# tnestmeyer/reflectance-filtering

Hardware: AMD Instinct MI355X
Metric: megapixels/sec joint-bilateral sigma_c=20 sigma_s=22 @1080p (higher is better)
Workload: dtype f32

## Files before the change

include/reflectance_filtering_debug.h:

```cpp
#ifndef REFLECTANCE_FILTERING_DEBUG_H
#define REFLECTANCE_FILTERING_DEBUG_H

#ifdef __cplusplus
extern "C" {
#endif

int rf_debug_option(const char *name, int value);

int rf_debug_clock_probe(unsigned long long *out2, int micros, void *stream);

const char *rf_debug_build_info(void);

int rf_debug_jbf_points_plan(int n_params, const double *sigma_space, int d, int joint_cn, int flags,
                             int total_points, int *out, int max_chunks);

int rf_debug_jbf_ragged_plan(int n, const int *heights, const int *widths, int joint_cn, int src_cn,
                             int d, double sigma_color, double sigma_space, int flags, int *out,
                             int cap);

int rf_debug_jbf_ragged_slab_plan(int n, const int *heights, const int *widths, int joint_cn,
                                  int src_cn, int d, double sigma_color, double sigma_space, int flags,
                                  int *out, int cap);

int rf_debug_jbf_two_wg_plan(int n, int h, int w, int joint_cn, int src_cn, int d, double sigma_color,
                             double sigma_space, int flags, int *out);

int rf_debug_jbf_two_wg_calls(void);

int rf_debug_jbf_tile_flags(void *stream, unsigned char *out, int cap);

int rf_debug_colorize_ragged_plan(int n, const int *heights, const int *widths, int *out, int cap);

int rf_debug_gf_ragged_plan(int n, const int *heights, const int *widths, int guide_cn, int src_cn,
                            int radius, int flags, int *out, int cap);

int rf_debug_gf_launch_chunk(int chunk, int h, int w, int src_cn, int float_kernels);

int rf_debug_png_plan(int n, const int *heights, const int *widths, int cn_in, int flags, int *out,
                      int cap);

#ifdef __cplusplus
}
#endif
#endif
```

reflectance_filtering_amd/_ffi.py:

```python
import ctypes
import os
import threading

_HERE = os.path.dirname(os.path.abspath(__file__))
LIB_PATH = os.path.join(_HERE, "librf_hip.so")

RF_OK, RF_E_BADARG, RF_E_UNSUPPORTED, RF_E_WORKSPACE, RF_E_HIP = 0, -1, -2, -3, -4
BORDER_CONSTANT, BORDER_REPLICATE, BORDER_REFLECT, BORDER_WRAP, BORDER_REFLECT_101 = range(5)
BORDER_DEFAULT = BORDER_REFLECT_101
JBF_TRUE_DIVISION = 1
JBF_FORCE_GENERIC = 2
JBF_GREY_AS_BGR = 4
GF_GREY_AS_BGR = 1
PNG_GREY_AS_RGB = 1
PNG_FLAG_GREY, PNG_FLAG_BAD_FILTER = 1, 2
CNN_NPARAMS = 4513
CNN_NPACKED = 4673
CNN_NCHW_RGB, CNN_NHWC_BGR = 0, 1
CNN_LAYOUTS = {"nchw_rgb": CNN_NCHW_RGB, "nhwc_bgr": CNN_NHWC_BGR}

EXPORTS = ("rf_version", "rf_last_error", "rf_shutdown", "rf_jbf_u8", "rf_gf_workspace_bytes",
           "rf_gf_u8", "rf_gf_ex_u8", "rf_cnn_reflectance_u8", "rf_cnn_pack_weights",
           "rf_cnn_reflectance_packed_u8", "rf_colorize_workspace_bytes",
           "rf_colorize_srgb_u8", "rf_whdr_f32", "rf_jbf_f32_workspace_bytes", "rf_jbf_f32",
           "rf_gf_f32_workspace_bytes", "rf_gf_f32", "rf_jbf_points_workspace_bytes",
           "rf_jbf_points_u8", "rf_jbf_points_ragged_workspace_bytes", "rf_jbf_points_ragged_u8",
           "rf_whdr_points_u8", "rf_jbf_ragged_workspace_bytes", "rf_jbf_ragged_u8",
           "rf_colorize_ragged_workspace_bytes", "rf_colorize_ragged_srgb_u8",
           "rf_gf_ragged_workspace_bytes", "rf_gf_ragged_u8", "rf_png_stream_bound",
           "rf_png_workspace_bytes", "rf_png_deflate_ragged_u8",
           "rf_png_unfilter_workspace_bytes", "rf_png_unfilter_ragged_u8",
           "rf_colorize_ragged_r8_srgb_u8", "rf_cnn_reflectance_f32",
           "rf_cnn_reflectance_packed_f32", "rf_jbf_release_scratch")

DEBUG_EXPORTS = ("rf_debug_option", "rf_debug_clock_probe", "rf_debug_build_info",
                 "rf_debug_jbf_points_plan", "rf_debug_jbf_ragged_plan",
                 "rf_debug_jbf_ragged_slab_plan", "rf_debug_jbf_two_wg_plan",
                 "rf_debug_jbf_two_wg_calls", "rf_debug_jbf_tile_flags",
                 "rf_debug_colorize_ragged_plan",
                 "rf_debug_gf_ragged_plan", "rf_debug_gf_launch_chunk", "rf_debug_png_plan")
RESULT_CHANGING_OPTIONS = ("jbf_stage_only", "gf_exp_skip")

_lib = None
_lock = threading.Lock()


class RFError(RuntimeError):
    """A librf_hip.so entry point returned a negative code."""


def load_library():
    global _lib
    with _lock:
# ... 93 lines not shown
        lib.rf_debug_clock_probe.restype = ci
        lib.rf_debug_build_info.argtypes = []
        lib.rf_debug_build_info.restype = ctypes.c_char_p
        lib.rf_debug_jbf_points_plan.argtypes = [ci, vp, ci, ci, ci, ci, vp, ci]
        lib.rf_debug_jbf_points_plan.restype = ci
        lib.rf_debug_jbf_ragged_plan.argtypes = [ci, vp, vp, ci, ci, ci, cd, cd, ci, vp, ci]
        lib.rf_debug_jbf_ragged_plan.restype = ci
        lib.rf_debug_jbf_ragged_slab_plan.argtypes = [ci, vp, vp, ci, ci, ci, cd, cd, ci, vp, ci]
        lib.rf_debug_jbf_ragged_slab_plan.restype = ci
        lib.rf_debug_jbf_two_wg_plan.argtypes = [ci, ci, ci, ci, ci, ci, cd, cd, ci, vp]
        lib.rf_debug_jbf_two_wg_plan.restype = ci
        lib.rf_debug_jbf_two_wg_calls.argtypes = []
        lib.rf_debug_jbf_two_wg_calls.restype = ci
        lib.rf_debug_jbf_tile_flags.argtypes = [vp, vp, ci]
        lib.rf_debug_jbf_tile_flags.restype = ci
        lib.rf_debug_colorize_ragged_plan.argtypes = [ci, vp, vp, vp, ci]
        lib.rf_debug_colorize_ragged_plan.restype = ci
        lib.rf_debug_gf_ragged_plan.argtypes = [ci, vp, vp, ci, ci, ci, ci, vp, ci]
        lib.rf_debug_gf_ragged_plan.restype = ci
        lib.rf_debug_gf_launch_chunk.argtypes = [ci, ci, ci, ci, ci]
        lib.rf_debug_gf_launch_chunk.restype = ci
        import sys
        for item in filter(None, os.environ.get("RF_DEBUG_OPTIONS", "").split(",")):
            name, _, value = item.partition("=")
            name = name.strip()
            try:
                number = int(value or 1)
            except ValueError:
                raise RFError("RF_DEBUG_OPTIONS: %r is not an integer (option %r)" % (value, name))
            if lib.rf_debug_option(name.encode(), number) < 0:
# ... 108 lines not shown
    return tuple(int(v) for v in out[1:]) if rc == 1 else None


def jbf_tile_flags(stream, tiles):
    import numpy as np
    lib = load_library()
    out = np.zeros(int(tiles), dtype=np.uint8)
    rc = lib.rf_debug_jbf_tile_flags(stream, out.ctypes.data, int(tiles))
    if rc < 0:
        check(rc, "rf_debug_jbf_tile_flags")
    if rc != int(tiles):
        raise RFError("rf_debug_jbf_tile_flags: %d bytes where %d tiles were asked for" % (rc, tiles))
    return out


def colorize_ragged_plan(sizes):
    import numpy as np
    lib = load_library()
    sizes = np.asarray(sizes, dtype=np.int64).reshape(-1, 2)
    n = sizes.shape[0]
    hs = np.ascontiguousarray(sizes[:, 0], dtype=np.int32)
    ws = np.ascontiguousarray(sizes[:, 1], dtype=np.int32)
    out = np.zeros(n + 2, dtype=np.int32)
    rc = lib.rf_debug_colorize_ragged_plan(n, hs.ctypes.data, ws.ctypes.data, out.ctypes.data, n + 2)
    if rc < 0:
        check(rc, "rf_debug_colorize_ragged_plan")
    return int(out[0]), int(out[1]), [int(v) for v in out[2:]]


def gf_ragged_plan(sizes, guide_cn, src_cn, radius, flags=0):
# ... 42 lines not shown
```

reflectance_filtering_amd/csrc/rf_api.hip:

```cpp
#include "rf_common.hpp"

#include <atomic>
#include <cstring>

#include "reflectance_filtering_debug.h"

namespace rf {

void jbf_shutdown();
void jbf_scratch_release();
void cnn_shutdown();
void gf_shutdown();

char *last_error_buf()
{
    static thread_local char buf[512] = "";
    return buf;
}

int fail(int code, const char *fmt, ...)
{
    va_list ap;
    va_start(ap, fmt);
    vsnprintf(last_error_buf(), 512, fmt, ap);
// ... 9 lines not shown

extern "C" int rf_debug_option(const char *name, int value)
{
    static const char *const names[] = {"gf_two_kernel",     "jbf_stage_only",
                                                      "jbf_compiler_loop", "jbf_tile64_only",
                                                      "jbf_tune",          "jbf_f32_untiled",
                                                      "cnn_lds_columns",   "gf_seg_rows",
                                                      "gf_one_stream",     "gf_force_two_streams",
                                                      "gf_guide_cache",    "gf_chained",        "gf_no_compact",
                                                      "gf_exp_skip",       "gf_stagger",        "gf_parts",
                                                      "gf_s1_cap",         "gf_s1_min_wgs",
                                                      "jbf_lookahead1",    "gf_s1_legacy_strips",
                                                      "gf_exact_all_flagged", "gf_cw_chan_run",   "gf_exact",
                                                      "jbf_no_msad",       "colorize_chunk_px",
                                                      "jbf_no_two_wg",     "jbf_vote_scan",
                                                      "jbf_no_dead_skip"};
    static_assert(sizeof(names) / sizeof(names[0]) == rf::kDbgCount, "one name per DebugOption");
    if (name)
        for (int i = 0; i < rf::kDbgCount; i++)
            if (std::strcmp(name, names[i]) == 0)
                return rf::g_debug[i].exchange(value < 0 ? 0 : value);
    return rf::fail(RF_E_BADARG, "rf_debug_option: unknown option '%s'", name ? name : "(null)");
}

__global__ void clock_probe_kernel(unsigned long long *out, unsigned long long ticks)
{
    if (threadIdx.x != 0)
        return;
    const unsigned long long r0 = __builtin_amdgcn_s_memrealtime();
    const unsigned long long c0 = __builtin_amdgcn_s_memtime();
    unsigned long long r1 = r0;
// ... 42 lines not shown
```

reflectance_filtering_amd/csrc/rf_common.hpp:

```cpp
#pragma once
#include <hip/hip_runtime.h>

#include <cstdarg>
#include <cstdint>
#include <cstdio>

#include "reflectance_filtering.h"

namespace rf {

char *last_error_buf();
int fail(int code, const char *fmt, ...);

#define RF_HIP_CHECK(expr)                                                                   \
    do {                                                                                     \
        hipError_t _e = (expr);                                                              \
        if (_e != hipSuccess)                                                                \
            return ::rf::fail(RF_E_HIP, "%s failed: %s (%s:%d)", #expr, hipGetErrorString(_e), \
                              __FILE__, __LINE__);                                           \
    } while (0)

__host__ __device__ inline int border_interpolate(int p, int len, int border)
{
    if ((unsigned)p < (unsigned)len)
// ... 69 lines not shown
    kDbgGfExpSkip,
    kDbgGfStagger,
    kDbgGfParts,
    kDbgGfS1Cap,
    kDbgGfS1MinWgs,
    kDbgJbfLookahead1,
    kDbgGfS1LegacyStrips,
    kDbgGfExactAllFlagged,
    kDbgGfCwChanRun,
    kDbgGfExact,
    kDbgJbfNoMsad,
    kDbgColorizeChunkPx,
    kDbgJbfNoTwoWg,
    kDbgJbfVoteScan,
    kDbgJbfNoDeadSkip,
    kDbgCount
};
int debug_get(int id);

}
```

reflectance_filtering_amd/csrc/rf_jbf.hip:

```cpp
#include <algorithm>
#include <atomic>
#include <mutex>
#include <vector>

#include "rf_jbf_common.hpp"
#include "rf_jbf_tables.hpp"
#include "rf_jbf_taploops.hpp"

namespace rf {
namespace {

constexpr int kTileW = 64;
constexpr int kMaxLds = 160 * 1024;
constexpr int kTlw2 = 144;
constexpr int kJbfMaxTiledR4 = 468;
constexpr int kJbfStageOnly = 0x1000, kJbfCompilerLoop = 0x2000, kJbfTile64Only = 0x4000;
constexpr int kJbfLookahead1 = 0x8000;
constexpr int kJbfNoMsad = 0x10000;
constexpr int kJbfVoteOnly = 0x20000;
constexpr int kJbfNoDeadSkip = 0x40000;

int jbf_debug_flags()
{
    return (debug_get(kDbgJbfStageOnly) ? kJbfStageOnly : 0) |
// ... 1074 lines not shown
    auto kern = jbf_slab_kernel<GREP, TLW, true>;
    RF_HIP_CHECK(hipFuncSetAttribute((const void *)kern, hipFuncAttributeMaxDynamicSharedMemorySize,
                                     kT64Lds));
    hipLaunchKernelGGL(kern, dim3((unsigned)ntiles), dim3(1024), kT64Lds, stream, joint, src, dst, 0,
                       0, jcn, scn, t.radius, border, t.d_lut, nz, t.d_hw, t.d_swsym, t.sw_len,
                       d_recs, 0, flags, s.crows_g, s.slab_g, s.crows_c, s.slab_c);
    return RF_OK;
}

int tile64x2_slab_rows(int nz, int grep, int tlw)
{
    const int rows = (kT64x2Lds - nz * grep * 4) / (tlw * 4);
    return rows >= 64 ? rows - 64 + 1 : 0;
}

template <int GREP, int TLW>
__global__ __launch_bounds__(1024, 8) void jbf_tile64x2_kernel(
    const uint8_t *__restrict__ joint, const uint8_t *__restrict__ src, uint8_t *__restrict__ dst,
    int h, int w, int jcn, int scn, int radius, int border, const float *__restrict__ lut, int nz,
    const int *__restrict__ hwtab, const float *__restrict__ swsym, int sw_len, int tiles_x,
    int tiles_per_img, int flags, int slab_rows, uint8_t *__restrict__ tile_flags)
{
    constexpr int NT = 1024, Q4 = TLW / 4, QW = 16;
    static_assert(TLW % 32 == 16, "row pitch keeps the rows of a half-wave on disjoint banks");
    extern __shared__ __align__(16) unsigned char smem[];
    int *flag_word = reinterpret_cast<int *>(smem);
    uint32_t *tile4 = reinterpret_cast<uint32_t *>(smem);
    const int tid = threadIdx.x;
    if (tid == 0)
        *flag_word = 3;
    __syncthreads();
    const int tile_id = xcd_contiguous_tile((int)blockIdx.x, (int)gridDim.x);
    const int img_idx = tile_id / tiles_per_img;
    const int t_in_img = tile_id - img_idx * tiles_per_img;
    const int tile_y0 = (t_in_img / tiles_x) * 64;
    const int tile_x0 = (t_in_img % tiles_x) * 64;
// ... 25 lines not shown
    if (tile_flags) {
        const int byte = __builtin_amdgcn_readfirstlane((int)tile_flags[tile_id]);
        if (byte & 1)
            return;
        grey_joint = (byte >> 1) & 1;
    }
    float *lut_g = reinterpret_cast<float *>(smem + kT64x2Lds - nz * GREP * 4);
    for (int i = tid; i < nz * GREP; i += NT)
        lut_g[i] = lut[i / GREP];
    const uint32_t lut_lane_addr = lds_addr(lut_g) + (uint32_t)(tid & (GREP - 1)) * 4u;
    const uint32_t tile_lane_addr = lds_addr(tile4) + (uint32_t)tx * 4u;
    const bool j1 = grey_joint != 0;
    const uint32_t j1_scale = (uint32_t)(jcn == 1 ? 1 : 3) * (GREP * 4u);
    uint32_t jc[kPix];
    float sum1[kPix][1], wsum[kPix];
    {
        uint32_t jv[4], sv[4];
        load_tile_quad(joint, src, img, border_interpolate(tile_y0 + ty, h, border), tile_x0 + 4 * tx, w, jcn,
                       scn, border, jv, sv);
#pragma unroll
        for (int p = 0; p < kPix; p++) {
            jc[p] = j1 ? (jv[p] & 0xffu) * j1_scale : jv[p] & 0x00ffffffu;
            sum1[p][0] = 0.f;
            wsum[p] = 0.f;
        }
    }
    const bool msad = !j1 && !(flags & kJbfNoMsad) && jbf_wave_takes_msad(jc);
    const bool live_wave =
        __builtin_amdgcn_readfirstlane(tile_y0 + (ty & ~3)) < h || (flags & kJbfNoDeadSkip) != 0;
    for (int i0 = -radius; i0 <= radius; i0 += slab_rows) {
        const int i1 = min(i0 + slab_rows - 1, radius);
        const int tlh = 64 + (i1 - i0);
        __syncthreads();
        for (int item = tid; item < tlh * Q4; item += NT) {
            const int ry = item / Q4, k = item - ry * Q4;
            const int gy = border_interpolate(tile_y0 + i0 + ry, h, border);
            uint32_t jv[4], sv[4];
            load_tile_quad(joint, src, img, gy, tile_x0 - r4 + 4 * k, w, jcn, scn, border, jv, sv);
#pragma unroll
            for (int u = 0; u < 4; u++) {
                const uint32_t jfield = j1 ? (jv[u] & 0xffu) * j1_scale : jv[u];
                tile4[ry * TLW + u * Q4 + k] = jfield | (sv[u] << 24);
            }
        }
        __syncthreads();
        if (!live_wave)
            continue;
        if (j1)
            jbf_tap_loop_grey4_la2<GREP, TLW, true, true>(lut_lane_addr, swsym, tile_lane_addr, jc, ty,
                                                          radius, r4, sw_len, hwtab, sum1, wsum, i0, i1, -i0);
        else if (msad)
            jbf_tap_loop_grey4_la2<GREP, TLW, false, true, true>(lut_lane_addr, swsym, tile_lane_addr, jc,
                                                                 ty, radius, r4, sw_len, hwtab, sum1, wsum,
                                                                 i0, i1, -i0);
        else
            jbf_tap_loop_grey4_la2<GREP, TLW, false, true>(lut_lane_addr, swsym, tile_lane_addr, jc, ty,
                                                           radius, r4, sw_len, hwtab, sum1, wsum, i0, i1,
// ... 4 lines not shown
    else
        store_quad<1, 3>(dst, img, tile_y0 + ty, tile_x0 + 4 * tx, h, w, sum1, wsum, flags);
}

struct TileFlagBuf {
    int dev;
    hipStream_t stream;
    uint8_t *p;
    size_t bytes;
};
std::mutex g_tf_mu;
std::vector<TileFlagBuf> g_tf;
std::vector<uint8_t *> g_tf_retired;
constexpr size_t kTileFlagStreams = 16;
std::atomic<int> g_two_wg_calls{0};

size_t tile_flag_bytes(size_t tiles)
{
    size_t b = 4096;
    while (b < tiles)
        b <<= 1;
    return b;
}

int get_tile_flags(int dev, hipStream_t stream, size_t tiles, uint8_t **out)
{
    *out = nullptr;
    std::lock_guard<std::mutex> lock(g_tf_mu);
    size_t at = g_tf.size();
    for (size_t i = 0; i < g_tf.size(); i++)
// ... 12 lines not shown
        return RF_OK;
    uint8_t *p = nullptr;
    {
        CaptureRelax relax;
        RF_HIP_CHECK(hipMalloc(&p, tile_flag_bytes(tiles)));
    }
    if (at < g_tf.size()) {
        g_tf_retired.push_back(g_tf[at].p);
        g_tf.erase(g_tf.begin() + at);
    }
    g_tf.push_back(TileFlagBuf{dev, stream, p, tile_flag_bytes(tiles)});
    *out = p;
    return RF_OK;
}

bool two_wg_choose(const JbfTables &t, int nz, int src_cn, int flags, int *slab_rows)
{
    *slab_rows = 0;
    if (debug_get(kDbgJbfNoTwoWg) || debug_get(kDbgJbfTune) ||
        (flags & (RF_JBF_FORCE_GENERIC | kJbfStageOnly | kJbfCompilerLoop | kJbfLookahead1)))
        return false;
    Tile64Shape shape;
    if (t.r4 > 36 || !tile64_choose(t, nz, src_cn, flags, &shape) || shape.tlw != 144 || shape.grep != 32)
        return false;
    *slab_rows = tile64x2_slab_rows(nz, 32, 144);
    return *slab_rows >= 8;
}

int launch_tile64x2(const JbfTables &t, int nz, int slab_rows, const uint8_t *joint, const uint8_t *src,
                    uint8_t *dst, int n, int h, int w, int jcn, int scn, int border, int flags,
                    hipStream_t stream, int rows, int cols, uint8_t *tile_flags)
{
    const int tiles_x = ceil_div(cols, 64), tiles_y = ceil_div(rows, 64);
    const long long blocks = (long long)tiles_x * tiles_y * n;
    auto kern = jbf_tile64x2_kernel<32, 144>;
    RF_HIP_CHECK(hipFuncSetAttribute((const void *)kern, hipFuncAttributeMaxDynamicSharedMemorySize,
                                     kT64x2Lds));
    hipLaunchKernelGGL(kern, dim3((unsigned)blocks), dim3(1024), kT64x2Lds, stream, joint, src, dst, h, w,
                       jcn, scn, t.radius, border, t.d_lut, nz, t.d_hw, t.d_swsym, t.sw_len, tiles_x,
                       tiles_x * tiles_y, flags, slab_rows, tile_flags);
    return RF_OK;
}

template <int CREP>
int launch_tile64_flagged(const JbfTables &t, int nz, int crows, const uint8_t *joint, const uint8_t *src,
                          uint8_t *dst, int n, int h, int w, int jcn, int border, int flags,
                          hipStream_t stream, int rows, int cols, const uint8_t *tile_flags)
{
    const int tiles_x = ceil_div(cols, 64), tiles_y = ceil_div(rows, 64);
    const long long blocks = (long long)tiles_x * tiles_y * n;
    auto kern = jbf_tile64_kernel<3, 32, CREP, 144, 64, false, true>;
    RF_HIP_CHECK(hipFuncSetAttribute((const void *)kern, hipFuncAttributeMaxDynamicSharedMemorySize,
                                     kT64Lds));
    hipLaunchKernelGGL(kern, dim3((unsigned)blocks), dim3(1024), kT64Lds, stream, joint, src, dst, h, w,
                       jcn, t.radius, border, t.d_lut, nz, t.d_hw, t.d_swsym, t.sw_len, tiles_x,
// ... 1 lines not shown
    return RF_OK;
}

int launch_two_wg(const JbfTables &t, int nz, const Tile64Shape &shape, int slab_rows,
                  const uint8_t *joint, const uint8_t *src, uint8_t *dst, int n, int h, int w, int jcn,
                  int scn, int border, int flags, hipStream_t stream, bool *done)
{
    *done = false;
    const Tile64Areas a = tile64_areas(t, nz, shape.grep, shape.crep, scn, flags, h, w);
    if (a.rows_main <= 0 || a.cols_main <= 0)
        return RF_OK;
    const long long blocks = (long long)ceil_div(a.cols_main, 64) * ceil_div(a.rows_main, 64) * n;
    if (!launch_fits(blocks, 1024))
        return fail(RF_E_UNSUPPORTED, "rf_jbf_u8: batch too large for one launch");
    uint8_t *tile_flags = nullptr;
    int rc = RF_OK;
    if (scn == 3 || jcn == 3) {
        if (int bad = get_tile_flags(t.device, stream, (size_t)blocks, &tile_flags))
            return bad;
        if (!tile_flags)
            return RF_OK;
        const int tiles_x = ceil_div(a.cols_main, 64), tiles_y = ceil_div(a.rows_main, 64);
        if (debug_get(kDbgJbfVoteScan) || !jbf_grey_map_serves(h, w, t.radius, border, tiles_x, tiles_y))
            rc = launch_tile64x2(t, nz, slab_rows, joint, src, dst, n, h, w, jcn, scn, border,
                                 flags | kJbfVoteOnly, stream, a.rows_main, a.cols_main, tile_flags);
        else
            rc = jbf_launch_grey_map(joint, src, n, h, w, jcn, scn, t.radius, border, stream, tiles_x, tiles_y,
                                     tile_flags);
    }
    if (rc == RF_OK && scn == 3)
        rc = shape.crep == 32 ? launch_tile64_flagged<32>(t, nz, shape.crows, joint, src, dst, n, h, w, jcn,
                                                          border, flags, stream, a.rows_main, a.cols_main,
                                                          tile_flags)
                              : launch_tile64_flagged<16>(t, nz, shape.crows, joint, src, dst, n, h, w, jcn,
                                                          border, flags, stream, a.rows_main, a.cols_main,
                                                          tile_flags);
    if (rc == RF_OK)
        rc = launch_tile64x2(t, nz, slab_rows, joint, src, dst, n, h, w, jcn, scn, border, flags, stream,
                             a.rows_main, a.cols_main, tile_flags);
    if (rc == RF_OK && (a.s32 || a.s16 || a.sx)) {
        if (scn == 3)
            rc = shape.crep == 32 ? launch_tile64_rows<3, 32, 32>(t, nz, shape.crows, joint, src, dst, n, h, w,
                                                                  jcn, border, flags, stream, true)
                                  : launch_tile64_rows<3, 32, 16>(t, nz, shape.crows, joint, src, dst, n, h, w,
                                                                  jcn, border, flags, stream, true);
        else
            rc = shape.crep == 32 ? launch_tile64_rows<1, 32, 32>(t, nz, shape.crows, joint, src, dst, n, h, w,
                                                                  jcn, border, flags, stream, true)
                                  : launch_tile64_rows<1, 32, 16>(t, nz, shape.crows, joint, src, dst, n, h, w,
                                                                  jcn, border, flags, stream, true);
    }
    *done = rc == RF_OK;
    if (*done)
        g_two_wg_calls.fetch_add(1, std::memory_order_relaxed);
    return rc;
}

}

void jbf_scratch_release()
{
    std::lock_guard<std::mutex> lock(g_tf_mu);
    for (const TileFlagBuf &b : g_tf)
        (void)hipFree(b.p);
    for (uint8_t *p : g_tf_retired)
        (void)hipFree(p);
    g_tf.clear();
    g_tf_retired.clear();
}

}

extern "C" int rf_debug_jbf_two_wg_calls(void)
{
    return rf::g_two_wg_calls.load(std::memory_order_relaxed) & 0x7fffffff;
}

extern "C" int rf_debug_jbf_tile_flags(void *stream_, unsigned char *out, int cap)
{
    using namespace rf;
    hipStream_t stream = (hipStream_t)stream_;
    if (cap < 0 || (!out && cap))
        return fail(RF_E_BADARG, "rf_debug_jbf_tile_flags: NULL out or a negative cap");
// ... 5 lines not shown
    const uint8_t *p = nullptr;
    size_t bytes = 0;
    {
        std::lock_guard<std::mutex> lock(g_tf_mu);
        for (const TileFlagBuf &b : g_tf)
            if (b.dev == dev && b.stream == stream)
                p = b.p, bytes = b.bytes;
    }
    if (bytes > (size_t)cap)
        bytes = (size_t)cap;
    if (bytes) {
        RF_HIP_CHECK(hipMemcpyAsync(out, p, bytes, hipMemcpyDeviceToHost, stream));
        RF_HIP_CHECK(hipStreamSynchronize(stream));
    }
    return (int)bytes;
}

extern "C" int rf_jbf_release_scratch(void)
{
    rf::jbf_scratch_release();
    return RF_OK;
}

extern "C" int rf_jbf_u8(const uint8_t *joint, const uint8_t *src, uint8_t *dst, int n, int h,
                         int w, int joint_cn, int src_cn, int d, double sigma_color,
                         double sigma_space, int border, int flags, void *stream_)
{
    using namespace rf;
    if (n == 0)
        return RF_OK;
// ... 265 lines not shown
    out[0] = out[1] = out[2] = out[3] = 0;
    int slab_rows = 0;
    Tile64Shape shape;
    if (t.r4 > kJbfMaxTiledR4 || !two_wg_choose(t, nz, src_cn, flags, &slab_rows) ||
        !tile64_choose(t, nz, src_cn, flags, &shape))
        return 0;
    const Tile64Areas a = tile64_areas(t, nz, shape.grep, shape.crep, src_cn, flags, h, w);
    const long long blocks = (long long)ceil_div(a.cols_main, 64) * ceil_div(a.rows_main, 64) * n;
    if (a.rows_main <= 0 || a.cols_main <= 0 || !launch_fits(blocks, 1024))
        return 0;
    out[0] = 1;
    out[1] = 64 + slab_rows - 1;
    out[2] = (int)blocks;
    out[3] = src_cn == 3 || joint_cn == 3 ? (int)tile_flag_bytes((size_t)blocks) : 0;
    return 1;
}

extern "C" int rf_jbf_ragged_u8(const uint8_t *joint, const uint8_t *src, uint8_t *dst, int n,
                                const int *heights, const int *widths, int joint_cn, int src_cn,
                                int d, double sigma_color, double sigma_space, int border, int flags,
                                void *workspace, size_t workspace_bytes, void *stream_)
{
    using namespace rf;
    const char *who = "rf_jbf_ragged_u8";
    if (n == 0)
        return RF_OK;
    if (!joint || !src || !dst)
        return fail(RF_E_BADARG, "%s: NULL image pointer", who);
    size_t px, tiles;
    if (int bad = ragged_check(who, n, heights, widths, joint_cn, src_cn, d, sigma_space, border,
// ... 91 lines not shown
```

reflectance_filtering_amd/csrc/rf_jbf_common.hpp:

```cpp
#pragma once
#include <cmath>
#include <vector>

#include "rf_common.hpp"

namespace rf {

constexpr int kJbfPublicFlags = RF_JBF_TRUE_DIVISION | RF_JBF_FORCE_GENERIC | RF_JBF_GREY_AS_BGR;
constexpr int kJbfMaxRadius = 4096;

inline double jbf_sigma(double sigma) { return sigma <= 0 ? 1 : sigma; }

inline int jbf_radius(int d, double sigma_space)
{
    const int radius = d <= 0 ? (int)std::lrint(sigma_space * 1.5) : d / 2;
    return radius < 1 ? 1 : radius;
}

inline int jbf_table_cn(int joint_cn, int flags)
{
    return joint_cn == 1 && (flags & RF_JBF_GREY_AS_BGR) ? 3 : joint_cn;
}
inline int jbf_kernel_cn(int joint_cn, int flags)
{
// ... 1 lines not shown
}

inline int jbf_check_format(const char *who, int joint_cn, int src_cn, int border)
{
    if ((joint_cn != 1 && joint_cn != 3) || (src_cn != 1 && src_cn != 3))
        return fail(RF_E_UNSUPPORTED, "%s: channels must be 1 or 3 (joint %d, src %d)", who,
                    joint_cn, src_cn);
    if (border < 0 || border > 4)
        return fail(RF_E_UNSUPPORTED, "%s: border type %d", who, border);
    return RF_OK;
}

bool jbf_grey_map_serves(int h, int w, int radius, int border, int tiles_x, int tiles_y);
int jbf_launch_grey_map(const uint8_t *joint, const uint8_t *src, int n, int h, int w, int jcn, int scn,
                        int radius, int border, hipStream_t stream, int tiles_x, int tiles_y,
                        uint8_t *tile_flags);

int jbf_colour_lut(int joint_cn, double sigma_color, std::vector<float> &lut);

void jbf_space_taps(int radius, double sigma_space, std::vector<int> &di, std::vector<int> &dj,
                    std::vector<float> &sw, std::vector<int> &hw);

__device__ inline uint32_t load_packed(const uint8_t *img, size_t pix, int cn)
{
    if (cn < 0)
        return (uint32_t)img[pix] * 0x010101u;
    const uint8_t *p = img + pix * cn;
    uint32_t v = p[0];
    if (cn == 3)
        v |= ((uint32_t)p[1] << 8) | ((uint32_t)p[2] << 16);
    return v;
// ... 16 lines not shown
```

reflectance_filtering_amd/csrc/rf_jbf_greymap.hip:

```cpp
#include "rf_jbf_common.hpp"

namespace rf {
namespace {

__host__ __device__ inline void border_span(int a, int b, int len, int border, int *lo, int *hi)
{
    int l = a > 0 ? a : 0, u = b < len - 1 ? b : len - 1;
    if (border == RF_BORDER_REFLECT || border == RF_BORDER_REFLECT_101) {
        const int delta = border == RF_BORDER_REFLECT_101;
        if (a < 0) {
            const int top = -a - 1 + delta;
            u = top > u ? (top < len - 1 ? top : len - 1) : u;
        }
        if (b >= len) {
            const int back = 2 * len - 1 - b - delta;
            l = back < l ? (back > 0 ? back : 0) : l;
        }
    }
    *lo = l;
    *hi = u;
}

constexpr int kMapCols = 10, kMapRows = 4, kMapColFirst = -2, kMapRowFirst = -1;
constexpr int kMapBatch = 4;
// ... 9 lines not shown

__device__ inline void load12(const uint8_t *p, uint32_t (&d)[3])
{
    __builtin_memcpy(&d[0], p, 4);
    __builtin_memcpy(&d[1], p + 4, 4);
    __builtin_memcpy(&d[2], p + 8, 4);
}

__device__ inline void load_row_end(const uint8_t *p, int npx, uint32_t (&d)[3])
{
    d[0] = d[1] = d[2] = 0u;
    for (int k = 0; k < 3 * npx; k++)
        d[k >> 2] |= (uint32_t)p[k] << (8 * (k & 3));
}

__global__ __launch_bounds__(256) void jbf_grey_map_clear_kernel(uint32_t *__restrict__ words, int nwords)
{
    const int i = (int)blockIdx.x * 256 + (int)threadIdx.x;
    if (i < nwords)
        words[i] = 0x02020202u;
}

template <bool SRC, bool JOINT>
__global__ __launch_bounds__(256) void jbf_grey_map_kernel(
    const uint8_t *__restrict__ joint, const uint8_t *__restrict__ src, int h, int w, int radius, int border,
    int tiles_x, int tiles_y, int blocks_x, int blocks_y, uint32_t *__restrict__ tile_words)
{
    __shared__ uint32_t acc[2 * kMapRows];
    const int tid = threadIdx.x, lane = tid & 63, wave = tid >> 6;
    if (tid < 2 * kMapRows)
        acc[tid] = 0u;
    const int gx = (int)(blockIdx.x % (unsigned)blocks_x);
    const int gy = (int)((blockIdx.x / (unsigned)blocks_x) % (unsigned)blocks_y);
    const int img_idx = (int)(blockIdx.x / ((unsigned)blocks_x * (unsigned)blocks_y));
    const int r4 = (radius + 3) & ~3;
    const int x = 256 * gx + 4 * lane;
    uint32_t cm[4] = {0u, 0u, 0u, 0u};
#pragma unroll
    for (int c = 0; c < kMapCols; c++) {
        const int tx = 4 * gx + kMapColFirst + c;
        if (tx < 0 || tx >= tiles_x)
            continue;
// ... 2 lines not shown
#pragma unroll
        for (int u = 0; u < 4; u++)
            cm[u] |= (x + u >= lo && x + u <= hi) ? 1u << c : 0u;
    }
    int ylo[kMapRows], yhi[kMapRows];
#pragma unroll
    for (int r = 0; r < kMapRows; r++) {
        const int ty = gy + kMapRowFirst + r;
        ylo[r] = 1, yhi[r] = 0;
        if (ty >= 0 && ty < tiles_y)
            border_span(64 * ty - radius, 64 * ty + 63 + radius, h, border, &ylo[r], &yhi[r]);
    }
    __syncthreads();
    uint32_t as[kMapRows] = {0u, 0u, 0u, 0u}, aj[kMapRows] = {0u, 0u, 0u, 0u};
    const size_t img = (size_t)img_idx * h * w;
    const bool active = (cm[0] | cm[1] | cm[2] | cm[3]) != 0u;
    if (active && w - x >= 4) {
        for (int i0 = 0; i0 < 16; i0 += kMapBatch) {
            const int y0 = 64 * gy + wave + 4 * i0;
            if (y0 >= h)
                break;
            uint32_t ds[kMapBatch][3], dj[kMapBatch][3];
#pragma unroll
            for (int k = 0; k < kMapBatch; k++) {
                const int yc = min(y0 + 4 * k, h - 1);
                const size_t at = (img + (size_t)yc * w + x) * 3;
                if (SRC)
                    load12(src + at, ds[k]);
                if (JOINT)
                    load12(joint + at, dj[k]);
            }
#pragma unroll
            for (int k = 0; k < kMapBatch; k++) {
                const int y = y0 + 4 * k;
                const uint32_t cs = SRC ? coloured_columns(ds[k], cm) : 0u;
                const uint32_t cj = JOINT ? coloured_columns(dj[k], cm) : 0u;
#pragma unroll
                for (int r = 0; r < kMapRows; r++)
                    if (y >= ylo[r] && y <= yhi[r])
                        as[r] |= cs, aj[r] |= cj;
            }
        }
    } else if (active) {
        for (int i = 0; i < 16; i++) {
            const int y = 64 * gy + wave + 4 * i;
            if (y >= h)
                break;
            const size_t at = (img + (size_t)y * w + x) * 3;
            uint32_t cs = 0u, cj = 0u, d[3];
            if (SRC) {
                load_row_end(src + at, w - x, d);
                cs = coloured_columns(d, cm);
            }
            if (JOINT) {
                load_row_end(joint + at, w - x, d);
                cj = coloured_columns(d, cm);
            }
#pragma unroll
            for (int r = 0; r < kMapRows; r++)
                if (y >= ylo[r] && y <= yhi[r])
                    as[r] |= cs, aj[r] |= cj;
        }
    }
#pragma unroll
    for (int r = 0; r < kMapRows; r++) {
        if (as[r])
            atomicOr(&acc[r], as[r]);
        if (aj[r])
            atomicOr(&acc[kMapRows + r], aj[r]);
    }
    __syncthreads();
// ... 25 lines not shown
            if (tx < 4 * gx + kMapColFirst || tx >= 4 * gx + kMapColFirst + kMapCols)
                return false;
    }
    for (int ty = 0; ty < tiles_y; ty++) {
        int lo, hi;
        border_span(64 * ty - radius, 64 * ty + 63 + radius, h, border, &lo, &hi);
        for (int gy = lo / 64; gy <= hi / 64; gy++)
            if (ty < gy + kMapRowFirst || ty >= gy + kMapRowFirst + kMapRows)
                return false;
    }
    return true;
}

int jbf_launch_grey_map(const uint8_t *joint, const uint8_t *src, int n, int h, int w, int jcn, int scn,
                        int radius, int border, hipStream_t stream, int tiles_x, int tiles_y,
                        uint8_t *tile_flags)
{
    const int blocks_x = ceil_div(w, 256), blocks_y = ceil_div(h, 64);
    const long long blocks = (long long)blocks_x * blocks_y * n;
    if (!launch_fits(blocks, 256))
        return fail(RF_E_UNSUPPORTED, "rf_jbf_u8: batch too large for one launch");
    const int nwords = (int)(((long long)tiles_x * tiles_y * n + 3) / 4);
    uint32_t *words = reinterpret_cast<uint32_t *>(tile_flags);
    hipLaunchKernelGGL(jbf_grey_map_clear_kernel, dim3((unsigned)ceil_div(nwords, 256)), dim3(256), 0, stream,
                       words, nwords);
    if (scn != 3 && jcn != 3)
        return RF_OK;
    auto kern = scn == 3 && jcn == 3 ? jbf_grey_map_kernel<true, true>
                : scn == 3           ? jbf_grey_map_kernel<true, false>
                                     : jbf_grey_map_kernel<false, true>;
    hipLaunchKernelGGL(kern, dim3((unsigned)blocks), dim3(256), 0, stream, joint, src, h, w, radius, border,
                       tiles_x, tiles_y, blocks_x, blocks_y, words);
    return RF_OK;
}

}
```

Before: 2727.

## Pack joint and source pixels into 32-bit texels during grey-map pass

The grey-map pre-pass, which already reads both 3-channel joint and source images, now also writes an intermediate buffer of 32-bit texels (joint BGR plus one source channel byte) with padded row pitch. The main two-workgroup tile kernel then fills its LDS tile from this buffer with aligned 16-byte loads instead of unaligned 3-byte-pixel gathers from two images. The aim is cheaper, vectorised tile staging. The cost is an extra global write pass in the pre-pass, a cached per-stream scratch allocation of up to 4 GB, and more code paths. It also changes the stage-only debug gating.

Result: no change. 2752 (median of 6 runs) (+0.9%).

```diff
diff --git a/include/reflectance_filtering_debug.h b/include/reflectance_filtering_debug.h
--- a/include/reflectance_filtering_debug.h
+++ b/include/reflectance_filtering_debug.h
@@ -29,6 +29,13 @@
 
 int rf_debug_jbf_tile_flags(void *stream, unsigned char *out, int cap);
 
+long long rf_debug_jbf_packed_plan(int n, int h, int w, int joint_cn, int src_cn, int d, double sigma_color,
+                                   double sigma_space, int border, int flags);
+
+int rf_debug_jbf_packed_calls(void);
+
+long long rf_debug_jbf_packed_texels(void *stream, unsigned int *out, long long cap);
+
 int rf_debug_colorize_ragged_plan(int n, const int *heights, const int *widths, int *out, int cap);
 
 int rf_debug_gf_ragged_plan(int n, const int *heights, const int *widths, int guide_cn, int src_cn,
diff --git a/reflectance_filtering_amd/_ffi.py b/reflectance_filtering_amd/_ffi.py
--- a/reflectance_filtering_amd/_ffi.py
+++ b/reflectance_filtering_amd/_ffi.py
@@ -37,6 +37,7 @@
                  "rf_debug_jbf_points_plan", "rf_debug_jbf_ragged_plan",
                  "rf_debug_jbf_ragged_slab_plan", "rf_debug_jbf_two_wg_plan",
                  "rf_debug_jbf_two_wg_calls", "rf_debug_jbf_tile_flags",
+                 "rf_debug_jbf_packed_plan", "rf_debug_jbf_packed_calls", "rf_debug_jbf_packed_texels",
                  "rf_debug_colorize_ragged_plan",
                  "rf_debug_gf_ragged_plan", "rf_debug_gf_launch_chunk", "rf_debug_png_plan")
 RESULT_CHANGING_OPTIONS = ("jbf_stage_only", "gf_exp_skip")
@@ -160,6 +161,12 @@
         lib.rf_debug_jbf_two_wg_calls.restype = ci
         lib.rf_debug_jbf_tile_flags.argtypes = [vp, vp, ci]
         lib.rf_debug_jbf_tile_flags.restype = ci
+        lib.rf_debug_jbf_packed_plan.argtypes = [ci, ci, ci, ci, ci, ci, cd, cd, ci, ci]
+        lib.rf_debug_jbf_packed_plan.restype = ctypes.c_longlong
+        lib.rf_debug_jbf_packed_calls.argtypes = []
+        lib.rf_debug_jbf_packed_calls.restype = ci
+        lib.rf_debug_jbf_packed_texels.argtypes = [vp, vp, ctypes.c_longlong]
+        lib.rf_debug_jbf_packed_texels.restype = ctypes.c_longlong
         lib.rf_debug_colorize_ragged_plan.argtypes = [ci, vp, vp, vp, ci]
         lib.rf_debug_colorize_ragged_plan.restype = ci
         lib.rf_debug_gf_ragged_plan.argtypes = [ci, vp, vp, ci, ci, ci, ci, vp, ci]
@@ -298,6 +305,29 @@
     return out
 
 
+def jbf_packed_plan(n, h, w, joint_cn, src_cn, d, sigma_color, sigma_space, border=None, flags=0):
+    lib = load_library()
+    rc = lib.rf_debug_jbf_packed_plan(int(n), int(h), int(w), int(joint_cn), int(src_cn), int(d),
+                                      float(sigma_color), float(sigma_space),
+                                      BORDER_DEFAULT if border is None else int(border), int(flags))
+    if rc < 0:
+        check(int(rc), "rf_debug_jbf_packed_plan")
+    return int(rc)
+
+
+def jbf_packed_texels(stream, n, h, w):
+    import numpy as np
+    lib = load_library()
+    wpad = (int(w) + 3) & ~3
+    out = np.zeros(int(n) * int(h) * wpad, dtype=np.uint32)
+    rc = lib.rf_debug_jbf_packed_texels(stream, out.ctypes.data, out.size)
+    if rc < 0:
+        check(int(rc), "rf_debug_jbf_packed_texels")
+    if rc != out.size:
+        return None
+    return np.ascontiguousarray(out.reshape(int(n), int(h), wpad)[:, :, :int(w)])
+
+
 def colorize_ragged_plan(sizes):
     import numpy as np
     lib = load_library()
diff --git a/reflectance_filtering_amd/csrc/rf_api.hip b/reflectance_filtering_amd/csrc/rf_api.hip
--- a/reflectance_filtering_amd/csrc/rf_api.hip
+++ b/reflectance_filtering_amd/csrc/rf_api.hip
@@ -47,7 +47,8 @@
                                                       "gf_exact_all_flagged", "gf_cw_chan_run",   "gf_exact",
                                                       "jbf_no_msad",       "colorize_chunk_px",
                                                       "jbf_no_two_wg",     "jbf_vote_scan",
-                                                      "jbf_no_dead_skip"};
+                                                      "jbf_no_dead_skip",  "jbf_no_packed",
+                                                      "jbf_packed_cap_kb"};
     static_assert(sizeof(names) / sizeof(names[0]) == rf::kDbgCount, "one name per DebugOption");
     if (name)
         for (int i = 0; i < rf::kDbgCount; i++)
diff --git a/reflectance_filtering_amd/csrc/rf_common.hpp b/reflectance_filtering_amd/csrc/rf_common.hpp
--- a/reflectance_filtering_amd/csrc/rf_common.hpp
+++ b/reflectance_filtering_amd/csrc/rf_common.hpp
@@ -107,6 +107,8 @@
     kDbgJbfNoTwoWg,
     kDbgJbfVoteScan,
     kDbgJbfNoDeadSkip,
+    kDbgJbfNoPacked,
+    kDbgJbfPackedCapKb,
     kDbgCount
 };
 int debug_get(int id);
diff --git a/reflectance_filtering_amd/csrc/rf_jbf.hip b/reflectance_filtering_amd/csrc/rf_jbf.hip
--- a/reflectance_filtering_amd/csrc/rf_jbf.hip
+++ b/reflectance_filtering_amd/csrc/rf_jbf.hip
@@ -1112,12 +1112,29 @@
     return rows >= 64 ? rows - 64 + 1 : 0;
 }
 
-template <int GREP, int TLW>
+__device__ inline void load_texel_quad(const uint32_t *row, int x_first, int w, int border, uint32_t (&t)[4])
+{
+    if (!row) {
+        t[0] = t[1] = t[2] = t[3] = 0u;
+    } else if (x_first >= 0 && x_first + 3 < w) {
+        const uint4 v = *reinterpret_cast<const uint4 *>(row + x_first);
+        t[0] = v.x, t[1] = v.y, t[2] = v.z, t[3] = v.w;
+    } else {
+#pragma unroll
+        for (int u = 0; u < 4; u++) {
+            const int gx = border_interpolate(x_first + u, w, border);
+            t[u] = gx < 0 ? 0u : row[gx];
+        }
+    }
+}
+
+template <int GREP, int TLW, bool PACKED = false>
 __global__ __launch_bounds__(1024, 8) void jbf_tile64x2_kernel(
     const uint8_t *__restrict__ joint, const uint8_t *__restrict__ src, uint8_t *__restrict__ dst,
     int h, int w, int jcn, int scn, int radius, int border, const float *__restrict__ lut, int nz,
     const int *__restrict__ hwtab, const float *__restrict__ swsym, int sw_len, int tiles_x,
-    int tiles_per_img, int flags, int slab_rows, uint8_t *__restrict__ tile_flags)
+    int tiles_per_img, int flags, int slab_rows, uint8_t *__restrict__ tile_flags,
+    const uint32_t *__restrict__ packed)
 {
     constexpr int NT = 1024, Q4 = TLW / 4, QW = 16;
     static_assert(TLW % 32 == 16, "row pitch keeps the rows of a half-wave on disjoint banks");
@@ -1173,6 +1190,8 @@
     const uint32_t j1_scale = (uint32_t)(jcn == 1 ? 1 : 3) * (GREP * 4u);
     uint32_t jc[kPix];
     float sum1[kPix][1], wsum[kPix];
+    const int wpad = (w + 3) & ~3;
+    const uint32_t *const pimg = PACKED ? packed + (size_t)img_idx * h * wpad : nullptr;
     {
         uint32_t jv[4], sv[4];
         load_tile_quad(joint, src, img, border_interpolate(tile_y0 + ty, h, border), tile_x0 + 4 * tx, w, jcn,
@@ -1184,22 +1203,40 @@
             wsum[p] = 0.f;
         }
     }
+    constexpr int kDry = NT / Q4, kDk = NT % Q4;
+    const int ry_first = tid / Q4, k_first = tid - ry_first * Q4;
     const bool msad = !j1 && !(flags & kJbfNoMsad) && jbf_wave_takes_msad(jc);
     const bool live_wave =
-        __builtin_amdgcn_readfirstlane(tile_y0 + (ty & ~3)) < h || (flags & kJbfNoDeadSkip) != 0;
+        (__builtin_amdgcn_readfirstlane(tile_y0 + (ty & ~3)) < h || (flags & kJbfNoDeadSkip) != 0) &&
+        !(flags & kJbfStageOnly);
     for (int i0 = -radius; i0 <= radius; i0 += slab_rows) {
         const int i1 = min(i0 + slab_rows - 1, radius);
         const int tlh = 64 + (i1 - i0);
         __syncthreads();
-        for (int item = tid; item < tlh * Q4; item += NT) {
-            const int ry = item / Q4, k = item - ry * Q4;
-            const int gy = border_interpolate(tile_y0 + i0 + ry, h, border);
-            uint32_t jv[4], sv[4];
-            load_tile_quad(joint, src, img, gy, tile_x0 - r4 + 4 * k, w, jcn, scn, border, jv, sv);
-#pragma unroll
-            for (int u = 0; u < 4; u++) {
-                const uint32_t jfield = j1 ? (jv[u] & 0xffu) * j1_scale : jv[u];
-                tile4[ry * TLW + u * Q4 + k] = jfield | (sv[u] << 24);
+        if (PACKED) {
+            static_assert(kTileW % 4 == 0 && Q4 * 4 == TLW, "quads of the tile start at multiples of four");
+            for (int ry = ry_first, k = k_first; ry < tlh;) {
+                const int gy = border_interpolate(tile_y0 + i0 + ry, h, border);
+                uint32_t t[4];
+                load_texel_quad(gy < 0 ? nullptr : pimg + (size_t)gy * wpad, tile_x0 - r4 + 4 * k, w, border, t);
+#pragma unroll
+                for (int u = 0; u < 4; u++)
+                    tile4[ry * TLW + u * Q4 + k] = j1 ? ((t[u] & 0xffu) * j1_scale) | (t[u] & 0xff000000u) : t[u];
+                k += kDk, ry += kDry;
+                if (k >= Q4)
+                    k -= Q4, ry++;
+            }
+        } else {
+            for (int item = tid; item < tlh * Q4; item += NT) {
+                const int ry = item / Q4, k = item - ry * Q4;
+                const int gy = border_interpolate(tile_y0 + i0 + ry, h, border);
+                uint32_t jv[4], sv[4];
+                load_tile_quad(joint, src, img, gy, tile_x0 - r4 + 4 * k, w, jcn, scn, border, jv, sv);
+#pragma unroll
+                for (int u = 0; u < 4; u++) {
+                    const uint32_t jfield = j1 ? (jv[u] & 0xffu) * j1_scale : jv[u];
+                    tile4[ry * TLW + u * Q4 + k] = jfield | (sv[u] << 24);
+                }
             }
         }
         __syncthreads();
@@ -1234,6 +1271,7 @@
 std::vector<uint8_t *> g_tf_retired;
 constexpr size_t kTileFlagStreams = 16;
 std::atomic<int> g_two_wg_calls{0};
+std::atomic<int> g_packed_calls{0};
 
 size_t tile_flag_bytes(size_t tiles)
 {
@@ -1276,11 +1314,73 @@
     return RF_OK;
 }
 
+struct PackedBuf {
+    int dev;
+    hipStream_t stream;
+    uint32_t *p;
+    size_t bytes;
+};
+std::vector<PackedBuf> g_pk;
+std::vector<uint32_t *> g_pk_retired;
+constexpr size_t kPackedCapBytes = (size_t)4 << 30;
+
+size_t packed_cap_bytes()
+{
+    const int kb = debug_get(kDbgJbfPackedCapKb);
+    return kb > 0 ? (size_t)kb << 10 : kPackedCapBytes;
+}
+
+size_t packed_bytes(int n, int h, int w) { return (size_t)n * h * ((w + 3) & ~3) * 4; }
+
+bool packed_choose(int n, int h, int w, int jcn, int scn, int radius, int border, int tiles_x, int tiles_y)
+{
+    return jcn == 3 && scn == 3 && !debug_get(kDbgJbfNoPacked) && !debug_get(kDbgJbfVoteScan) &&
+           jbf_grey_map_serves(h, w, radius, border, tiles_x, tiles_y) &&
+           packed_bytes(n, h, w) <= packed_cap_bytes();
+}
+
+void get_packed(int dev, hipStream_t stream, size_t bytes, uint32_t **out)
+{
+    *out = nullptr;
+    std::lock_guard<std::mutex> lock(g_tf_mu);
+    size_t at = g_pk.size();
+    for (size_t i = 0; i < g_pk.size(); i++)
+        if (g_pk[i].dev == dev && g_pk[i].stream == stream)
+            at = i;
+    if (at < g_pk.size() && g_pk[at].bytes >= bytes) {
+        *out = g_pk[at].p;
+        return;
+    }
+    hipStreamCaptureStatus st = hipStreamCaptureStatusNone;
+    if (hipStreamIsCapturing(stream, &st) != hipSuccess || st != hipStreamCaptureStatusNone) {
+        (void)hipGetLastError();
+        return;
+    }
+    if (at == g_pk.size() && g_pk.size() >= kTileFlagStreams)
+        return;
+    uint32_t *p = nullptr;
+    {
+        CaptureRelax relax;
+        if (hipMalloc(&p, bytes) != hipSuccess) {
+            (void)hipGetLastError();
+            return;
+        }
+    }
+    if (at < g_pk.size()) {
+        g_pk_retired.push_back(g_pk[at].p);
+        g_pk.erase(g_pk.begin() + at);
+    }
+    g_pk.push_back(PackedBuf{dev, stream, p, bytes});
+    *out = p;
+}
+
 bool two_wg_choose(const JbfTables &t, int nz, int src_cn, int flags, int *slab_rows)
 {
     *slab_rows = 0;
     if (debug_get(kDbgJbfNoTwoWg) || debug_get(kDbgJbfTune) ||
-        (flags & (RF_JBF_FORCE_GENERIC | kJbfStageOnly | kJbfCompilerLoop | kJbfLookahead1)))
+        (flags & (RF_JBF_FORCE_GENERIC | kJbfCompilerLoop | kJbfLookahead1)))
+        return false;
+    if ((flags & kJbfStageOnly) && debug_get(kDbgJbfStageOnly) != 2)
         return false;
     Tile64Shape shape;
     if (t.r4 > 36 || !tile64_choose(t, nz, src_cn, flags, &shape) || shape.tlw != 144 || shape.grep != 32)
@@ -1291,16 +1391,17 @@
 
 int launch_tile64x2(const JbfTables &t, int nz, int slab_rows, const uint8_t *joint, const uint8_t *src,
                     uint8_t *dst, int n, int h, int w, int jcn, int scn, int border, int flags,
-                    hipStream_t stream, int rows, int cols, uint8_t *tile_flags)
+                    hipStream_t stream, int rows, int cols, uint8_t *tile_flags,
+                    const uint32_t *packed = nullptr)
 {
     const int tiles_x = ceil_div(cols, 64), tiles_y = ceil_div(rows, 64);
     const long long blocks = (long long)tiles_x * tiles_y * n;
-    auto kern = jbf_tile64x2_kernel<32, 144>;
+    auto kern = packed ? jbf_tile64x2_kernel<32, 144, true> : jbf_tile64x2_kernel<32, 144>;
     RF_HIP_CHECK(hipFuncSetAttribute((const void *)kern, hipFuncAttributeMaxDynamicSharedMemorySize,
                                      kT64x2Lds));
     hipLaunchKernelGGL(kern, dim3((unsigned)blocks), dim3(1024), kT64x2Lds, stream, joint, src, dst, h, w,
                        jcn, scn, t.radius, border, t.d_lut, nz, t.d_hw, t.d_swsym, t.sw_len, tiles_x,
-                       tiles_x * tiles_y, flags, slab_rows, tile_flags);
+                       tiles_x * tiles_y, flags, slab_rows, tile_flags, packed);
     return RF_OK;
 }
 
@@ -1332,6 +1433,7 @@
     if (!launch_fits(blocks, 1024))
         return fail(RF_E_UNSUPPORTED, "rf_jbf_u8: batch too large for one launch");
     uint8_t *tile_flags = nullptr;
+    uint32_t *packed = nullptr;
     int rc = RF_OK;
     if (scn == 3 || jcn == 3) {
         if (int bad = get_tile_flags(t.device, stream, (size_t)blocks, &tile_flags))
@@ -1342,9 +1444,12 @@
         if (debug_get(kDbgJbfVoteScan) || !jbf_grey_map_serves(h, w, t.radius, border, tiles_x, tiles_y))
             rc = launch_tile64x2(t, nz, slab_rows, joint, src, dst, n, h, w, jcn, scn, border,
                                  flags | kJbfVoteOnly, stream, a.rows_main, a.cols_main, tile_flags);
-        else
+        else {
+            if (packed_choose(n, h, w, jcn, scn, t.radius, border, tiles_x, tiles_y))
+                get_packed(t.device, stream, packed_bytes(n, h, w), &packed);
             rc = jbf_launch_grey_map(joint, src, n, h, w, jcn, scn, t.radius, border, stream, tiles_x, tiles_y,
-                                     tile_flags);
+                                     tile_flags, packed);
+        }
     }
     if (rc == RF_OK && scn == 3)
         rc = shape.crep == 32 ? launch_tile64_flagged<32>(t, nz, shape.crows, joint, src, dst, n, h, w, jcn,
@@ -1355,7 +1460,7 @@
                                                           tile_flags);
     if (rc == RF_OK)
         rc = launch_tile64x2(t, nz, slab_rows, joint, src, dst, n, h, w, jcn, scn, border, flags, stream,
-                             a.rows_main, a.cols_main, tile_flags);
+                             a.rows_main, a.cols_main, tile_flags, packed);
     if (rc == RF_OK && (a.s32 || a.s16 || a.sx)) {
         if (scn == 3)
             rc = shape.crep == 32 ? launch_tile64_rows<3, 32, 32>(t, nz, shape.crows, joint, src, dst, n, h, w,
@@ -1369,8 +1474,11 @@
                                                                   jcn, border, flags, stream, true);
     }
     *done = rc == RF_OK;
-    if (*done)
+    if (*done) {
         g_two_wg_calls.fetch_add(1, std::memory_order_relaxed);
+        if (packed)
+            g_packed_calls.fetch_add(1, std::memory_order_relaxed);
+    }
     return rc;
 }
 
@@ -1385,6 +1493,12 @@
         (void)hipFree(p);
     g_tf.clear();
     g_tf_retired.clear();
+    for (const PackedBuf &b : g_pk)
+        (void)hipFree(b.p);
+    for (uint32_t *p : g_pk_retired)
+        (void)hipFree(p);
+    g_pk.clear();
+    g_pk_retired.clear();
 }
 
 }
@@ -1420,6 +1534,39 @@
         RF_HIP_CHECK(hipStreamSynchronize(stream));
     }
     return (int)bytes;
+}
+
+extern "C" int rf_debug_jbf_packed_calls(void)
+{
+    return rf::g_packed_calls.load(std::memory_order_relaxed) & 0x7fffffff;
+}
+
+extern "C" long long rf_debug_jbf_packed_texels(void *stream_, unsigned int *out, long long cap)
+{
+    using namespace rf;
+    hipStream_t stream = (hipStream_t)stream_;
+    if (cap < 0 || (!out && cap))
+        return fail(RF_E_BADARG, "rf_debug_jbf_packed_texels: NULL out or a negative cap");
+    if (stream_is_capturing(stream))
+        return fail(RF_E_UNSUPPORTED, "rf_debug_jbf_packed_texels: synchronises its stream and cannot be "
+                                      "captured into a graph");
+    int dev = 0;
+    RF_HIP_CHECK(hipGetDevice(&dev));
+    const uint32_t *p = nullptr;
+    size_t texels = 0;
+    {
+        std::lock_guard<std::mutex> lock(g_tf_mu);
+        for (const PackedBuf &b : g_pk)
+            if (b.dev == dev && b.stream == stream)
+                p = b.p, texels = b.bytes / 4;
+    }
+    if (texels > (size_t)cap)
+        texels = (size_t)cap;
+    if (texels) {
+        RF_HIP_CHECK(hipMemcpyAsync(out, p, texels * 4, hipMemcpyDeviceToHost, stream));
+        RF_HIP_CHECK(hipStreamSynchronize(stream));
+    }
+    return (long long)texels;
 }
 
 extern "C" int rf_jbf_release_scratch(void)
@@ -1715,6 +1862,31 @@
     out[2] = (int)blocks;
     out[3] = src_cn == 3 || joint_cn == 3 ? (int)tile_flag_bytes((size_t)blocks) : 0;
     return 1;
+}
+
+extern "C" long long rf_debug_jbf_packed_plan(int n, int h, int w, int joint_cn, int src_cn, int d,
+                                              double sigma_color, double sigma_space, int border, int flags)
+{
+    using namespace rf;
+    int route[4];
+    const int rc = rf_debug_jbf_two_wg_plan(n, h, w, joint_cn, src_cn, d, sigma_color, sigma_space, flags, route);
+    if (rc < 0)
+        return rc;
+    if (int bad = jbf_check_format("rf_debug_jbf_packed_plan", joint_cn, src_cn, border))
+        return bad;
+    if (rc == 0)
+        return 0;
+    std::vector<float> lut;
+    const JbfTables t = jbf_host_tables(jbf_radius(d, jbf_sigma(sigma_space)), jbf_table_cn(joint_cn, flags),
+                                        jbf_sigma(sigma_color), jbf_sigma(sigma_space), lut);
+    const int nz = t.lut_len < 256 * t.joint_cn ? t.lut_len - 1 : t.lut_len;
+    Tile64Shape shape;
+    tile64_choose(t, nz, src_cn, flags | jbf_debug_flags(), &shape);
+    const Tile64Areas a = tile64_areas(t, nz, shape.grep, shape.crep, src_cn, flags | jbf_debug_flags(), h, w);
+    return packed_choose(n, h, w, jbf_kernel_cn(joint_cn, flags), src_cn, t.radius, border,
+                         ceil_div(a.cols_main, 64), ceil_div(a.rows_main, 64))
+               ? (long long)packed_bytes(n, h, w)
+               : 0;
 }
 
 extern "C" int rf_jbf_ragged_u8(const uint8_t *joint, const uint8_t *src, uint8_t *dst, int n,
diff --git a/reflectance_filtering_amd/csrc/rf_jbf_common.hpp b/reflectance_filtering_amd/csrc/rf_jbf_common.hpp
--- a/reflectance_filtering_amd/csrc/rf_jbf_common.hpp
+++ b/reflectance_filtering_amd/csrc/rf_jbf_common.hpp
@@ -39,7 +39,7 @@
 bool jbf_grey_map_serves(int h, int w, int radius, int border, int tiles_x, int tiles_y);
 int jbf_launch_grey_map(const uint8_t *joint, const uint8_t *src, int n, int h, int w, int jcn, int scn,
                         int radius, int border, hipStream_t stream, int tiles_x, int tiles_y,
-                        uint8_t *tile_flags);
+                        uint8_t *tile_flags, uint32_t *packed);
 
 int jbf_colour_lut(int joint_cn, double sigma_color, std::vector<float> &lut);
 
diff --git a/reflectance_filtering_amd/csrc/rf_jbf_greymap.hip b/reflectance_filtering_amd/csrc/rf_jbf_greymap.hip
--- a/reflectance_filtering_amd/csrc/rf_jbf_greymap.hip
+++ b/reflectance_filtering_amd/csrc/rf_jbf_greymap.hip
@@ -47,6 +47,14 @@
         d[k >> 2] |= (uint32_t)p[k] << (8 * (k & 3));
 }
 
+__device__ inline void pack_texels(const uint32_t (&dj)[3], const uint32_t (&ds)[3], uint32_t (&t)[4])
+{
+    t[0] = (dj[0] & 0x00ffffffu) | (ds[0] << 24);
+    t[1] = (dj[0] >> 24) | ((dj[1] & 0xffffu) << 8) | (ds[0] & 0xff000000u);
+    t[2] = (dj[1] >> 16) | ((dj[2] & 0xffu) << 16) | ((ds[1] << 8) & 0xff000000u);
+    t[3] = (dj[2] >> 8) | ((ds[2] << 16) & 0xff000000u);
+}
+
 __global__ __launch_bounds__(256) void jbf_grey_map_clear_kernel(uint32_t *__restrict__ words, int nwords)
 {
     const int i = (int)blockIdx.x * 256 + (int)threadIdx.x;
@@ -54,11 +62,13 @@
         words[i] = 0x02020202u;
 }
 
-template <bool SRC, bool JOINT>
+template <bool SRC, bool JOINT, bool PACK = false>
 __global__ __launch_bounds__(256) void jbf_grey_map_kernel(
     const uint8_t *__restrict__ joint, const uint8_t *__restrict__ src, int h, int w, int radius, int border,
-    int tiles_x, int tiles_y, int blocks_x, int blocks_y, uint32_t *__restrict__ tile_words)
-{
+    int tiles_x, int tiles_y, int blocks_x, int blocks_y, uint32_t *__restrict__ tile_words,
+    uint32_t *__restrict__ packed)
+{
+    static_assert(!PACK || (SRC && JOINT), "a texel is packed from two 3-channel buffers");
     __shared__ uint32_t acc[2 * kMapRows];
     const int tid = threadIdx.x, lane = tid & 63, wave = tid >> 6;
     if (tid < 2 * kMapRows)
@@ -91,7 +101,9 @@
     __syncthreads();
     uint32_t as[kMapRows] = {0u, 0u, 0u, 0u}, aj[kMapRows] = {0u, 0u, 0u, 0u};
     const size_t img = (size_t)img_idx * h * w;
-    const bool active = (cm[0] | cm[1] | cm[2] | cm[3]) != 0u;
+    const bool active = (cm[0] | cm[1] | cm[2] | cm[3]) != 0u || (PACK && x < w);
+    const int wpad = (w + 3) & ~3;
+    const size_t prow0 = (size_t)img_idx * h;
     if (active && w - x >= 4) {
         for (int i0 = 0; i0 < 16; i0 += kMapBatch) {
             const int y0 = 64 * gy + wave + 4 * i0;
@@ -116,6 +128,11 @@
                 for (int r = 0; r < kMapRows; r++)
                     if (y >= ylo[r] && y <= yhi[r])
                         as[r] |= cs, aj[r] |= cj;
+                if (PACK && y < h) {
+                    uint32_t t[4];
+                    pack_texels(dj[k], ds[k], t);
+                    *reinterpret_cast<uint4 *>(packed + (prow0 + y) * wpad + x) = make_uint4(t[0], t[1], t[2], t[3]);
+                }
             }
         }
     } else if (active) {
@@ -124,14 +141,20 @@
             if (y >= h)
                 break;
             const size_t at = (img + (size_t)y * w + x) * 3;
-            uint32_t cs = 0u, cj = 0u, d[3];
+            uint32_t cs = 0u, cj = 0u, d[3], e[3];
             if (SRC) {
-                load_row_end(src + at, w - x, d);
-                cs = coloured_columns(d, cm);
+                load_row_end(src + at, w - x, e);
+                cs = coloured_columns(e, cm);
             }
             if (JOINT) {
                 load_row_end(joint + at, w - x, d);
                 cj = coloured_columns(d, cm);
+            }
+            if (PACK) {
+                uint32_t t[4];
+                pack_texels(d, e, t);
+                for (int u = 0; u < w - x; u++)
+                    packed[(prow0 + y) * wpad + x + u] = t[u];
             }
 #pragma unroll
             for (int r = 0; r < kMapRows; r++)
@@ -187,8 +210,10 @@
 
 int jbf_launch_grey_map(const uint8_t *joint, const uint8_t *src, int n, int h, int w, int jcn, int scn,
                         int radius, int border, hipStream_t stream, int tiles_x, int tiles_y,
-                        uint8_t *tile_flags)
-{
+                        uint8_t *tile_flags, uint32_t *packed)
+{
+    if (scn != 3 || jcn != 3)
+        packed = nullptr;
     const int blocks_x = ceil_div(w, 256), blocks_y = ceil_div(h, 64);
     const long long blocks = (long long)blocks_x * blocks_y * n;
     if (!launch_fits(blocks, 256))
@@ -199,11 +224,12 @@
                        words, nwords);
     if (scn != 3 && jcn != 3)
         return RF_OK;
-    auto kern = scn == 3 && jcn == 3 ? jbf_grey_map_kernel<true, true>
-                : scn == 3           ? jbf_grey_map_kernel<true, false>
-                                     : jbf_grey_map_kernel<false, true>;
+    auto kern = packed                 ? jbf_grey_map_kernel<true, true, true>
+                : scn == 3 && jcn == 3 ? jbf_grey_map_kernel<true, true>
+                : scn == 3             ? jbf_grey_map_kernel<true, false>
+                                       : jbf_grey_map_kernel<false, true>;
     hipLaunchKernelGGL(kern, dim3((unsigned)blocks), dim3(256), 0, stream, joint, src, h, w, radius, border,
-                       tiles_x, tiles_y, blocks_x, blocks_y, words);
+                       tiles_x, tiles_y, blocks_x, blocks_y, words, packed);
     return RF_OK;
 }
 
```
